# kleinzcy/speech_signal_processing

Measured on AMD Instinct MI355X. Metric: MFCC frames/s (one fused pass: framing .. DCT + delta + delta-delta, 39-d), higher is better.
Workload: dtype f32; 1 GPU; configs[1]: 100000 x 3 s synthetic 16 kHz utterances per GPU, 39-d MFCC (+delta+delta-delta), 400/160/512, 24 mel; utterances_per_gpu=100000, frames_per_gpu=29800000, d_out=39, parallelism=utterance-sharded x1, world_size_observed=1

## Files before the change

### speech_signal_processing_amd/csrc/mfcc.hpp

```cpp
#pragma once
#include "common.hpp"

namespace ssp {

struct MfccChunk {
    int32_t utt;
    int32_t t0;
    int32_t n;
    int32_t pad;
};

struct MfccArgs {
    const float* samples;
    const int64_t* sample_off;
    const int64_t* frame_off;
    float* out;
    float* lm_out;
    const MfccChunk* chunks;
    float* utt_max;
    const float* window;
    const float2* twiddle;
    const int32_t* filt_lo4;
    const float* filt_wT;
    const int32_t* filt_grp;
    int32_t filt_w4_total;
    int32_t dct_identity;
    int32_t dct_ncp;
    const float* dct;
    const float* dctT;
    int32_t win_len, hop, n_fft, n_filt, n_ceps, d_out;
    int32_t frame_mode, preemph_mode, spec_power, log_mode, floor_mode, delta_order, delta_N, cmvn;
    float preemph, spec_scale, eps, top_db, delta_inv_denom;
    int32_t lds_logmel_off, lds_ceps_off, lds_dlt_off, lds_ddl_off, lds_lmrows_off, lds_stats_off, lds_tw_off;
    int32_t lds_dct_off;
    int32_t lds_wt_off;
    int32_t lm_stride;
    int32_t n_chunks;
    int32_t prefetch;
};

constexpr int MFCC_FAST_MAX_PASS = 4;

struct FastArgs {
    const float2* tw16;
    const float2* wpost;
    const float* melw;
    const int32_t* mel_lo;
    const int32_t* mel_id;
    const float* dctT;
    int32_t mel_steps[MFCC_FAST_MAX_PASS];
    int32_t mel_blocks[MFCC_FAST_MAX_PASS];
    int32_t lm_pad;
    int32_t n_pass, q_pass, total_steps, n_filt4;
    float ddw[17];
    int32_t slen;
    int32_t stage_floats;
    int32_t ceps_rows;
    int32_t off_win, off_tw16, off_wpost, off_melw, off_mello, off_melid, off_dct, off_ceps, off_stats, off_wave, wave_bytes;
    float pscale;
    float one_minus_a;
    const float* pc_w;
    const int32_t* pc_ofs;
    const float* pc_mask;
    const int32_t* pc_fid;
    int32_t melv;
    int32_t mel_ns;
    float log_add, log_max, log_k;
    float* ceps_scratch;
    int32_t* work_counter;
    int32_t* redo_flags;
    int32_t ceps_stride;
    int32_t n_chunks;
};

struct StreamArgs {
    const float* dctA;
    int32_t* work_counter;
    int32_t* redo_flags;
    int32_t n_chunks;
    int32_t wave_bytes;
    int32_t stage_bytes;
    int32_t table_bytes;
    int32_t tstep;
    const float* dense_w;
};

int launch_mfcc_generic(const MfccArgs& args, int n_chunks, size_t lds_bytes, int n_waves, int num_cu, hipStream_t stream);
int launch_cmvn(const float* in, float* out, const int64_t* frame_off_dev, int64_t n_utt, int dim, int64_t max_T, hipStream_t stream);
int launch_topdb_dct(const float* logmel, const int64_t* frame_off_dev, int64_t n_utt, const MfccChunk* chunks, int n_chunks,
                     const float* utt_max, int n_filt, int n_ceps, const float* dct, float top_db, float* out, hipStream_t stream);
    

}

struct ssp_mfcc_plan {
    ssp_ctx* ctx = nullptr;
    ssp_mfcc_cfg cfg{};
    int32_t d_out = 0;
    bool reproducible = false;
    ssp::DevBuf window, twiddle, filt_lo4, filt_grp, filt_wT, dct, dctT, fbank_dense;
    int32_t max_filt_len = 0;
    uint64_t checked_sseg = 0, checked_fseg = 0;
    uint64_t cache_sseg = 0;
    uint64_t cache_fseg = 0;
    int cache_variant = -1;
    int cache_request = -1;
    bool cache_split_cmvn = false;
    bool cache_split_topdb = false;
    ssp::DevBuf lm_scratch, umax_scratch;
    int cache_chunk_frames = 0;
    size_t cache_lds = 0;
    int cache_waves = 4;
    int32_t cache_n_chunks = 0;
    std::vector<int32_t> cache_chunk_first;
    ssp::DevBuf chunks;
    ssp::MfccArgs args{};
    bool fast_ready = false;
    int64_t fast_max_samples = 0;
    ssp::FastArgs fast{};
    ssp::DevBuf f_tw16, f_wpost, f_melw, f_mello, f_melid, f_dct, f_pcw, f_pcofs, f_pcmask, f_pcfid, f_scratch, f_counter;
    bool stream_ready = false;
    ssp::DevBuf s_dctA, s_dense;
    bool cache_s2k_fused = false;
    bool s2k_ready = false;
    int32_t s2k_steps = 0, s2k_steps1 = 0;
    ssp::DevBuf s2k_twA, s2k_twB, s2k_twS, s2k_mel, s2k_minfo;
};

namespace ssp {
bool mfcc_fast_supported(const ssp_mfcc_cfg& cfg);
int build_fast_tables(ssp_mfcc_plan* plan);
size_t mfcc_fast_lds(const ssp_mfcc_cfg& cfg, FastArgs& f, int chunk_frames);
int mfcc_fast_max_chunk(const ssp_mfcc_cfg& cfg, const FastArgs& f);
int launch_mfcc_fast(const MfccArgs& args, ssp_mfcc_plan* plan, int n_chunks, int chunk_frames, hipStream_t stream);
bool mfcc_stream_supported(const ssp_mfcc_plan* plan);
bool mfcc_s2k_supported(const ssp_mfcc_plan* plan);
int build_s2k_tables(ssp_mfcc_plan* plan);
bool mfcc_s2k_fuses(const ssp_mfcc_plan* plan, int64_t max_T, int chunk_frames);
int launch_mfcc_s2k(const MfccArgs& args, ssp_mfcc_plan* plan, int n_chunks, hipStream_t stream);
bool mfcc_stream_dense(const ssp_mfcc_plan* plan);
bool mfcc_stream_fuses_cmvn(const ssp_mfcc_plan* plan);
int build_stream_tables(ssp_mfcc_plan* plan);
int launch_mfcc_stream(const MfccArgs& args, ssp_mfcc_plan* plan, int n_chunks, hipStream_t stream, bool dry_run = false);
}
```

### speech_signal_processing_amd/csrc/mfcc_plan.hip

```cpp
#include <chrono>
#include <cmath>
#include <cstdlib>

#include "mfcc.hpp"

namespace ssp {

static int validate_cfg(const ssp_mfcc_cfg* c) {
    if (!c) SSP_FAIL(SSP_ERR_INVALID, "mfcc: null cfg");
    if (c->n_fft < 64 || c->n_fft > 2048 || (c->n_fft & (c->n_fft - 1)))
        SSP_FAIL(SSP_ERR_UNSUPPORTED, "mfcc: n_fft=%d must be a power of two in [64, 2048]", c->n_fft);
    if (c->win_len < 1 || c->win_len > c->n_fft) SSP_FAIL(SSP_ERR_INVALID, "mfcc: win_len=%d not in [1, n_fft]", c->win_len);
    if (c->hop < 1) SSP_FAIL(SSP_ERR_INVALID, "mfcc: hop < 1");
    if (c->n_filt < 1 || c->n_filt > 512) SSP_FAIL(SSP_ERR_INVALID, "mfcc: n_filt=%d not in [1,512]", c->n_filt);
    if (c->n_ceps < 1 || c->n_ceps > 128) SSP_FAIL(SSP_ERR_INVALID, "mfcc: n_ceps=%d not in [1,128]", c->n_ceps);
    if (c->frame_mode < 0 || c->frame_mode > 2) SSP_FAIL(SSP_ERR_INVALID, "mfcc: frame_mode");
    if (c->frame_mode == 2 && c->win_len != c->n_fft)
        SSP_FAIL(SSP_ERR_UNSUPPORTED, "mfcc: centred framing needs win_len == n_fft");
    if (c->preemph_mode < 0 || c->preemph_mode > 1) SSP_FAIL(SSP_ERR_INVALID, "mfcc: preemph_mode");
    if (c->spec_power != 1 && c->spec_power != 2) SSP_FAIL(SSP_ERR_INVALID, "mfcc: spec_power must be 1 or 2");
    if (c->log_mode < 0 || c->log_mode > 2) SSP_FAIL(SSP_ERR_INVALID, "mfcc: log_mode");
    if (c->floor_mode < 0 || c->floor_mode > 2) SSP_FAIL(SSP_ERR_INVALID, "mfcc: floor_mode");
    if (c->delta_order < 0 || c->delta_order > 2) SSP_FAIL(SSP_ERR_INVALID, "mfcc: delta_order must be 0, 1 or 2");
    if (c->delta_order > 0 && (c->delta_N < 1 || c->delta_N > 8))
// ... 124 lines not shown
        if (whole) {
            ch = (int)std::max<int64_t>(max_T, 1);
            if (generic_lds_layout(c, ch, 8, &tmp) <= lds_cap) {
                nw = 8;
            } else if (generic_lds_layout(c, ch, 4, &tmp) > lds_cap) {
                if (c.top_db >= 0.f) {
                    if (c.delta_order != 0 || c.cmvn)
                        SSP_FAIL(SSP_ERR_UNSUPPORTED,
                                 "mfcc: top_db with deltas / cmvn needs a whole utterance per workgroup; %lld frames exceed the 160 KiB LDS",
                                 (long long)max_T);
                    split_topdb = true;
                } else {
                    split_cmvn = true;
                }
                whole = false;
                ch = chunk_for(c);
                if (split_topdb) {
                    ssp_mfcc_cfg c2 = c;
                    c2.top_db = -1.f;
                    ch = chunk_for(c2);
                }
            }
        }
        {
            ssp_mfcc_cfg c2 = c;
            if (split_topdb) c2.top_db = -1.f;
            lds = generic_lds_layout(c2, ch, nw, &p->args);
        }
        if (lds > lds_cap) SSP_FAIL(SSP_ERR_UNSUPPORTED, "mfcc: LDS footprint %zu B exceeds 160 KiB", lds);
    }
    std::vector<MfccChunk> chunks;
    chunks.reserve((size_t)fseg->n);
    int64_t tail_from = fseg->n;
#ifndef SSP_NO_TAIL_SPLIT
    if (variant == 3 && !(c.cmvn != 0 && !split_cmvn) && !getenv("SSP_MFCC_NO_TAIL_SPLIT")) {
        const int64_t waves = (int64_t)p->ctx->num_cu * 12;
        if (fseg->n >= 4 * waves) tail_from = fseg->n - waves;
    }
#endif
    p->cache_chunk_first.assign((size_t)fseg->n + 1, 0);
    for (int64_t u = 0; u < fseg->n; ++u) {
        const int64_t T = fseg->host[u + 1] - fseg->host[u];
        if (T > INT32_MAX) SSP_FAIL(SSP_ERR_UNSUPPORTED, "mfcc: utterance %lld has too many frames", (long long)u);
        p->cache_chunk_first[(size_t)u] = (int32_t)std::min<size_t>(chunks.size(), (size_t)INT32_MAX);
        int64_t chu = ch;
        if (u >= tail_from && T >= 64) chu = std::min<int64_t>(ch, ((T + 1) / 2 + 15) / 16 * 16);
        const int pad = (variant == 3 && (!small_batch || repro)) ? 12 : 0;
        for (int64_t t0 = 0; t0 < T; t0 += chu)
            chunks.push_back(MfccChunk{(int32_t)u, (int32_t)t0, (int32_t)std::min<int64_t>(chu, T - t0), t0 > 0 ? pad : 0});
    }
    if (chunks.size() > (size_t)INT32_MAX) SSP_FAIL(SSP_ERR_UNSUPPORTED, "mfcc: too many chunks");
    p->cache_chunk_first[(size_t)fseg->n] = (int32_t)chunks.size();
    SSP_TRY(upload(p->chunks, chunks, p->ctx->stream));
    SSP_HIP(hipStreamSynchronize(p->ctx->stream));
    p->fast_max_samples = sseg->max_len();
    p->cache_n_chunks = (int32_t)chunks.size();
    p->cache_chunk_frames = ch;
    p->cache_lds = lds;
    p->cache_waves = nw;
    p->cache_sseg = sseg->serial;
    p->cache_fseg = fseg->serial;
    p->cache_variant = variant;
    p->cache_split_cmvn = split_cmvn;
    p->cache_split_topdb = split_topdb;
    return SSP_OK;
}

}

using namespace ssp;

extern "C" {

int ssp_mfcc_num_frames(const ssp_mfcc_cfg* cfg, int64_t n_samples, int64_t* n_frames) {
    if (!cfg || !n_frames || n_samples < 0) SSP_FAIL(SSP_ERR_INVALID, "ssp_mfcc_num_frames: bad argument");
    if (cfg->hop < 1 || cfg->frame_mode < 0 || cfg->frame_mode > 2) SSP_FAIL(SSP_ERR_INVALID, "ssp_mfcc_num_frames: bad cfg");
    *n_frames = frames_for(*cfg, n_samples);
    return SSP_OK;
}

int ssp_mfcc_out_dim(const ssp_mfcc_cfg* cfg, int32_t* d_out) {
    if (!cfg || !d_out) SSP_FAIL(SSP_ERR_INVALID, "ssp_mfcc_out_dim: null");
    *d_out = cfg->n_ceps * (1 + cfg->delta_order);
    return SSP_OK;
}

int ssp_mfcc_plan_create(ssp_ctx* ctx, const ssp_mfcc_cfg* cfg, const float* window, const float* fbank,
                         const float* dct, ssp_mfcc_plan** out) {
    ssp::TraceRange trace_("ssp_mfcc_plan_create");
    if (!out) SSP_FAIL(SSP_ERR_INVALID, "ssp_mfcc_plan_create: null out");
    *out = nullptr;
    SSP_TRY(use_ctx(ctx));
    SSP_TRY(validate_cfg(cfg));
    if (!window || !fbank || !dct) SSP_FAIL(SSP_ERR_INVALID, "ssp_mfcc_plan_create: null table");
    ssp_mfcc_plan* p = new (std::nothrow) ssp_mfcc_plan;
    if (!p) SSP_FAIL(SSP_ERR_NOMEM, "mfcc plan: host alloc");
    p->ctx = ctx;
    p->cfg = *cfg;
    p->d_out = cfg->n_ceps * (1 + cfg->delta_order);
    const int n_fft = cfg->n_fft, nb = n_fft / 2 + 1;

    std::vector<float> win(n_fft, 0.f);
    for (int i = 0; i < cfg->win_len; ++i) win[i] = window[i];
    std::vector<float2> tw(n_fft);
    for (int k = 0; k < n_fft; ++k) {
        const double ang = -2.0 * M_PI * (double)k / (double)n_fft;
// ... 523 lines not shown
```

### speech_signal_processing_amd/csrc/mfcc_stream_kernel.hpp

```cpp
#pragma once
#include <algorithm>
#include <cmath>
#include <cstdlib>
#include <type_traits>

#include "mfcc.hpp"
#include "cplx.hpp"

namespace ssp {

namespace {
typedef unsigned v2u __attribute__((ext_vector_type(2)));
typedef __attribute__((address_space(3))) const volatile v2f* lds_cv2f_t;
typedef __attribute__((address_space(3))) const volatile float* lds_cvf_t;
constexpr int ZROW = 128;
constexpr int ZFRAME = 16 * ZROW;
constexpr int LM_OFF = 1792;
constexpr int RING_FRAMES = 24;
constexpr int RING_ROW = 64;
constexpr int STREAM_WAVES = 4;
#ifndef SSP_S_PSHIFT
#define SSP_S_PSHIFT 64
#endif
constexpr int PSH = SSP_S_PSHIFT;
static_assert(4 * (256 + 24) + PSH <= LM_OFF - 192, "shifted P row: piece reads must stay below the log-mel rows");
#define SSP_STR_(x) #x
#define SSP_STR(x) SSP_STR_(x)

__device__ __forceinline__ float stream_log(const FastArgs& f, float v) {
    return __builtin_amdgcn_logf(fmaxf(v + f.log_add, f.log_max)) * f.log_k;
}

__device__ __forceinline__ float delta_weight(float t, float tp, float Tm1, float half_inv) {
    const float lo = tp <= 0.f ? -1.0e6f : tp;
    const float hi = tp >= Tm1 ? 1.0e6f : tp;
    const float a = fmaxf(lo, t - 2.f), b = fminf(hi, t + 2.f);
    const float cnt = fmaxf(b - a + 1.f, 0.f);
    const float w = cnt * (a + b - 2.f * t) * half_inv;
    return (tp < 0.f || tp > Tm1) ? 0.f : w;
}
}

template <int NZ, int POWER, int PRE, int MELV, int KS, int NS, int OCC, int CM, int WALK, int GEO>
__device__ __forceinline__ void mfcc_stream512_body(const MfccArgs& a, const FastArgs& f, const StreamArgs& sa) {
    static_assert(GEO >= 0 && GEO <= 3 && (GEO == 0 || (NZ == 13 && KS == 6 && MELV != 0)), "fixed geometry: the 400 / 160 / 24-filter family only");
    constexpr bool FIXG = GEO != 0;
    extern __shared__ __attribute__((aligned(16))) char smem[];
    if (WALK && sa.work_counter[1] == 0) return;
    const int tid = threadIdx.x, lane = tid & 63;
    const int wave = __builtin_amdgcn_readfirstlane(tid >> 6);
    const int g = lane >> 4, j = lane & 15;
    constexpr int nc = 13;
    constexpr int mel_ns = NS;

    char* zbuf = smem + wave * sa.wave_bytes;
    float* stage = reinterpret_cast<float*>(zbuf + 4 * ZFRAME);
    char* ring = zbuf + 4 * ZFRAME + sa.stage_bytes;

    v2f wreg[NZ];
#pragma unroll
    for (int n1 = 0; n1 < NZ; ++n1) wreg[n1] = *reinterpret_cast<const v2f*>(a.window + 32 * n1 + 2 * j);
#pragma unroll
    for (int n1 = 0; n1 < NZ; ++n1) wreg[n1] = edge_row_taps(wreg[n1], 32 * n1 + 2 * j, a.win_len);
#ifndef SSP_STREAM_NTW
#define SSP_STREAM_NTW 15
#endif
#ifndef SSP_STREAM_NTW_CM
#define SSP_STREAM_NTW_CM 12
#endif
#ifndef SSP_STREAM_NWP
#define SSP_STREAM_NWP 8
#endif
    constexpr int NTW = OCC >= 3 ? (CM ? SSP_STREAM_NTW_CM : ((MELV <= 3 && NS <= 2) ? SSP_STREAM_NTW : ((MELV >= 4 && NS >= 4) ? 8 : 9))) : 15, NWP = OCC >= 3 ? SSP_STREAM_NWP : 8;
    static_assert(NTW >= 8, "rows above NTW take W^((k1 - 8) j) W^(8 j): W^(8 j) = twr[7] must be resident");
    v2f twr[NTW], wpr[NWP];
#pragma unroll
    for (int k1 = 1; k1 <= NTW; ++k1) twr[k1 - 1] = *reinterpret_cast<const v2f*>(&f.tw16[k1 * 16 + j]);
    float dA[KS];
#pragma unroll
    for (int s = 0; s < KS; ++s) dA[s] = sa.dctA[s * 64 + lane];
#pragma unroll
    for (int i = 0; i < NWP; ++i) wpr[i] = *reinterpret_cast<const v2f*>(&f.wpost[i * 16 + j]);
    constexpr bool DENSE = MELV == 0;
    constexpr int MV = DENSE ? 1 : MELV;
    v4f mw[MV];
    int mofs[MV];
    v2f mk01 = v2f{0.f, 0.f}, mk23 = v2f{0.f, 0.f};
    int mfid = -1;
    v4f dw[DENSE ? 6 : 1][4];
    float dw256[DENSE ? 6 : 1];
    if (DENSE) {
#pragma unroll
        for (int k = 0; k < 6; ++k) {
#pragma unroll
            for (int i = 0; i < 4; ++i) dw[DENSE ? k : 0][i] = *reinterpret_cast<const v4f*>(sa.dense_w + ((size_t)lane * 6 + k) * 20 + 4 * i);
            dw256[DENSE ? k : 0] = sa.dense_w[((size_t)lane * 6 + k) * 20 + 16];
        }
    } else {
#pragma unroll
        for (int i = 0; i < MV; ++i) {
            mw[i] = *reinterpret_cast<const v4f*>(f.pc_w + ((size_t)lane * MV + i) * 4);
            mofs[i] = f.pc_ofs[lane * MV + i];
        }
        mk01 = *reinterpret_cast<const v2f*>(f.pc_mask + lane * 4);
        mk23 = NS > 2 ? *reinterpret_cast<const v2f*>(f.pc_mask + lane * 4 + 2) : v2f{0.f, 0.f};
        mfid = f.pc_fid[lane];
    }

    const int hop = FIXG ? 160 : a.hop;
    const float pre = PRE ? a.preemph : 0.f;
    const float npre = -pre;
    const int slen = FIXG ? 3 * 160 + 32 * 13 : f.slen;
    const int n_piece = (slen + 255) >> 8;
    const bool has_half = (slen & 255) != 0 && (slen & 255) <= 128;
    const int n_full = has_half ? n_piece - 1 : n_piece;
    const int dord = FIXG ? GEO - 1 : a.delta_order;
    const int Dd = FIXG ? nc * GEO : a.d_out;
    const int n_filt = FIXG ? 24 : a.n_filt;
    const int lm_pad = FIXG ? 0 : f.lm_pad;
    const float half_inv = 0.5f * a.delta_inv_denom;
    const uint32_t stage_lds = __builtin_amdgcn_readfirstlane((uint32_t)(uintptr_t)(lds_ptr_t)stage);

#ifdef SSP_S_CLOCK
    const unsigned long long ck0 = __builtin_amdgcn_s_memtime(), rt0 = __builtin_amdgcn_s_memrealtime();
#endif
    uint64_t wm = 0;
    int wblk = blockIdx.x * STREAM_WAVES + wave, wbase = 0;
    for (;;) {
        int cidx = 0;
        if constexpr (WALK) {
            bool done = false;
            while (wm == 0) {
                if ((int64_t)wblk * 64 >= sa.n_chunks) {
                    done = true;
                    break;
                }
                const int idx = wblk * 64 + lane;
                const int fl = idx < sa.n_chunks ? sa.redo_flags[idx] : 0;
                wm = __builtin_amdgcn_ballot_w64(fl != 0);
                wbase = wblk * 64;
                wblk += gridDim.x * STREAM_WAVES;
            }
            if (done) break;
            cidx = __builtin_amdgcn_readfirstlane(wbase + __builtin_ctzll(wm));
            wm &= wm - 1;
        } else {
            if (lane == 0) cidx = atomicAdd(sa.work_counter, 1);
            cidx = __builtin_amdgcn_readfirstlane(cidx);
            if (cidx >= sa.n_chunks) break;
        }
        const MfccChunk ch = a.chunks[cidx];
        const int64_t s0 = a.sample_off[ch.utt];
        const int64_t N = a.sample_off[ch.utt + 1] - s0;
        const int64_t f0 = a.frame_off[ch.utt];
        const int T = __builtin_amdgcn_readfirstlane((int)(a.frame_off[ch.utt + 1] - f0));
        const int t0 = __builtin_amdgcn_readfirstlane(ch.t0), n = __builtin_amdgcn_readfirstlane(ch.n);
        const int H = dord > 0 ? 4 : 0;
        const int Hlo = dord > 0 ? H + __builtin_amdgcn_readfirstlane(ch.pad) : 0;
        const int ta = max(t0 - Hlo, 0), tb = min(t0 + n + H, T);
        const int R = tb - ta;
        const int nquads = (R + 3) >> 2;
        const int E = t0 + n - ta;
        const int n_steps = (E + 4 + 15) >> 4;
        const int Q = DENSE ? nquads : 4 * n_steps;
        const float Tm1 = (float)(T - 1);

        const uint64_t xaddr = reinterpret_cast<uint64_t>(a.samples + s0);
        const uint32_t xlo = __builtin_amdgcn_readfirstlane((uint32_t)xaddr), xhi = __builtin_amdgcn_readfirstlane((uint32_t)(xaddr >> 32));
        const int xbytes = __builtin_amdgcn_readfirstlane((int)(N * 4));
        const __amdgpu_buffer_rsrc_t rs = __builtin_amdgcn_make_buffer_rsrc(
            reinterpret_cast<float*>(((uint64_t)xhi << 32) | xlo), 0, xbytes, 0x00020000);
        const uint64_t oaddr = reinterpret_cast<uint64_t>(a.out + (size_t)f0 * Dd);
        const uint32_t olo = __builtin_amdgcn_readfirstlane((uint32_t)oaddr), ohi = __builtin_amdgcn_readfirstlane((uint32_t)(oaddr >> 32));
        const __amdgpu_buffer_rsrc_t ro = __builtin_amdgcn_make_buffer_rsrc(
            reinterpret_cast<float*>(((uint64_t)ohi << 32) | olo), 0, __builtin_amdgcn_readfirstlane(T * Dd * 4), 0x00020000);

        auto prefetch = [&](int q) {
            int ol = lane;
            if (FIXG) asm volatile("" : "+v"(ol));
            const int vo = (ta + 4 * q) * hop * 4 + ol * 16;
            const lds_ptr_t lp = (lds_ptr_t)(uintptr_t)stage_lds;
            if (FIXG) {
                __builtin_amdgcn_raw_ptr_buffer_load_lds(rs, lp, 16, vo, 0, 0, 0);
                __builtin_amdgcn_raw_ptr_buffer_load_lds(rs, lp, 16, vo, 0, 1024, 0);
                __builtin_amdgcn_raw_ptr_buffer_load_lds(rs, lp, 16, vo, 0, 2048, 0);
                if (lane < 32) __builtin_amdgcn_raw_ptr_buffer_load_lds(rs, lp, 16, vo, 0, 3072, 0);
                return;
            }
            if (n_full > 0) __builtin_amdgcn_raw_ptr_buffer_load_lds(rs, lp, 16, vo, 0, 0, 0);
            if (n_full > 1) __builtin_amdgcn_raw_ptr_buffer_load_lds(rs, lp, 16, vo, 0, 1024, 0);
            if (n_full > 2) __builtin_amdgcn_raw_ptr_buffer_load_lds(rs, lp, 16, vo, 0, 2048, 0);
            if (n_full > 3) __builtin_amdgcn_raw_ptr_buffer_load_lds(rs, lp, 16, vo, 0, 3072, 0);
            if (n_full > 4) __builtin_amdgcn_raw_ptr_buffer_load_lds(rs, (lds_ptr_t)(uintptr_t)(stage_lds + 4096), 16, vo + 4096, 0, 0, 0);
            if (has_half && lane < 32)
                __builtin_amdgcn_raw_ptr_buffer_load_lds(rs, (lds_ptr_t)(uintptr_t)(stage_lds + n_full * 1024), 16, vo + n_full * 1024, 0, 0, 0);
        };

        {
            float zz = 0.f;
            asm volatile("" : "+v"(zz));
            v4f z4 = v4f{zz, zz, zz, zz};
            *reinterpret_cast<v4f*>(ring + lane * 16) = z4;
            if (lane < (RING_FRAMES * RING_ROW - 1024) / 16) *reinterpret_cast<v4f*>(ring + 1024 + lane * 16) = z4;
        }
        prefetch(0);
        int stores_pending = 0;
        int cm_nf = WALK;
        float cs1[CM ? 3 : 1] = {}, cs2[CM ? 3 : 1] = {};
        float piv = 0.f;

        typedef v2f zarr_t[16];
        typedef v2f pfarr_t[NZ];
        typedef float pmarr_t[PRE ? NZ : 1];
        constexpr int NH = (NZ + 1) / 2;
        auto wait_dma = [&]() {
#ifndef SSP_S_NOWAIT
            if constexpr (FIXG) {
                if (__builtin_expect(stores_pending == 0, 1)) {
                    asm volatile("s_waitcnt vmcnt(0)" ::: "memory");
                } else {
                    int np = stores_pending;
                    asm volatile("" : "+s"(np));
// ... 126 lines not shown
                        if (POWER == 1) {
                            pa[u] = __builtin_amdgcn_sqrtf(pa[u]);
                            pb[u] = __builtin_amdgcn_sqrtf(pb[u]);
                        }
                    }
                    const int k2 = 2 * kp;
                    P[j + 16 * k2] = pa[0];
                    P[j + 16 * (k2 + 1)] = pa[1];
                    Pm[16 * (6 - k2)] = pb[1];
                    Pm[16 * (7 - k2)] = pb[0];
                }
                const v2f s8 = z[8] * z[8];
                float p128 = 4.f * (s8.x + s8.y);
                if (POWER == 1) p128 = __builtin_amdgcn_sqrtf(p128);
                if (j == 0) P[128] = p128;
            }
        };
        auto mel = [&]() {
#ifndef SSP_S_NOMEL
            if (!CM) {
                float* lm = reinterpret_cast<float*>(zbuf + g * ZFRAME + LM_OFF - 64 * g);
                if (j < lm_pad) lm[n_filt + j] = 0.f;
            } else if (j < lm_pad) {
                int ol = lane;
                asm volatile("" : "+v"(ol));
                reinterpret_cast<float*>(zbuf + (ol >> 4) * (ZFRAME - 64) + LM_OFF)[n_filt + (ol & 15)] = 0.f;
            }
            float sfr[4];
#pragma unroll
            for (int fr = 0; fr < 4; ++fr) {
                const char* pr = zbuf + fr * ZFRAME + (fr & 1) * PSH;
                v4f acc = *reinterpret_cast<const v4f*>(pr + mofs[0]) * mw[0];
#pragma unroll
                for (int i = 1; i < MV; ++i) acc = __builtin_elementwise_fma(*reinterpret_cast<const v4f*>(pr + mofs[i]), mw[i], acc);
                const v2f h = v2f{acc.x, acc.y} + v2f{acc.z, acc.w};
                sfr[fr] = h.x + h.y;
            }
            v2f s01 = v2f{sfr[0], sfr[1]}, s23 = v2f{sfr[2], sfr[3]};
#define SSP_SCAN_STEP(CTRL, MK)                                                                     \
            {                                                                                           \
                const float a0 = s01.x, a1 = s01.y, a2 = s23.x, a3 = s23.y;                             \
                const float b0 = __builtin_amdgcn_update_dpp(a0, a0, CTRL, 0xF, 0xF, true);           \
                const float b1 = __builtin_amdgcn_update_dpp(a1, a1, CTRL, 0xF, 0xF, true);           \
                const float b2 = __builtin_amdgcn_update_dpp(a2, a2, CTRL, 0xF, 0xF, true);           \
                const float b3 = __builtin_amdgcn_update_dpp(a3, a3, CTRL, 0xF, 0xF, true);           \
                s01 = __builtin_elementwise_fma(v2f{b0, b1}, MK, s01);                                  \
                s23 = __builtin_elementwise_fma(v2f{b2, b3}, MK, s23);                                  \
            }
            if (mel_ns > 0) SSP_SCAN_STEP(0x101 , xx(mk01))
            if (mel_ns > 1) SSP_SCAN_STEP(0x102 , yy(mk01))
            if (mel_ns > 2) SSP_SCAN_STEP(0x104 , xx(mk23))
            if (mel_ns > 3) SSP_SCAN_STEP(0x108 , yy(mk23))
#undef SSP_SCAN_STEP
            if (mfid >= 0) {
                float* lmf = reinterpret_cast<float*>(zbuf + LM_OFF) + mfid;
                lmf[0 * (ZFRAME - 64) / 4] = stream_log(f, s01.x);
                lmf[1 * (ZFRAME - 64) / 4] = stream_log(f, s01.y);
                lmf[2 * (ZFRAME - 64) / 4] = stream_log(f, s23.x);
                lmf[3 * (ZFRAME - 64) / 4] = stream_log(f, s23.y);
            }
#endif
        };
        auto dct_mfma = [&]() -> v4f {
            v4f cq = v4f{0.f, 0.f, 0.f, 0.f};
#ifndef SSP_S_NODCT
            int ol = lane;
            asm volatile("" : "+v"(ol));
            const int g = ol >> 4, j = ol & 15;
            const char* lmrow = zbuf + (j & 3) * (ZFRAME - 64) + LM_OFF + g * (KS * 4);
            float lb[KS];
#pragma unroll
            for (int s = 0; s < KS; s += 2) {
                const v2f v = *reinterpret_cast<const v2f*>(lmrow + 4 * s);
                lb[s] = v.x;
                lb[s + 1] = v.y;
            }
#pragma unroll
            for (int s = 0; s < KS; ++s) cq = __builtin_amdgcn_mfma_f32_16x16x4f32(dA[s], lb[s], cq, 0, 0, 0);
#endif
            return cq;
        };
        constexpr int RING_BYTES = RING_FRAMES * RING_ROW, QROW = 4 * RING_ROW;
        auto ring_wrap = [](int o) { return o >= RING_BYTES ? o - RING_BYTES : o; };
        int qrow = 0, srow = 0;
        auto ring_put = [&](int qq, v4f cq, bool real) {
            int ol = lane;
            asm volatile("" : "+v"(ol));
            const int g = ol >> 4, j = ol & 15;
            if (j < 4) {
                const bool ok = real && ta + 4 * qq + j < tb;
                const v4f cv = ok ? cq : v4f{0.f, 0.f, 0.f, 0.f};
                if constexpr (FIXG) *reinterpret_cast<v4f*>(ring + qrow + j * RING_ROW + g * 16) = cv;
                else *reinterpret_cast<v4f*>(ring + ((((qq + 6) % 6) * 4 + j) * RING_ROW) + g * 16) = cv;
            }
            if (FIXG) qrow = ring_wrap(qrow + QROW);
        };
        typedef float cbarr_t[6];
        auto ring_window = [&](int b, cbarr_t& cb) {
            const int rb = 16 * b;
            int ol = lane;
            asm volatile("" : "+v"(ol));
            const int g = ol >> 4, j = ol & 15;
            int mb = ring_wrap(srow + 16 * RING_ROW);
#pragma unroll
            for (int s = 0; s < 6; ++s) {
                if constexpr (FIXG) {
                    cb[s] = *reinterpret_cast<const float*>(ring + mb + g * RING_ROW + j * 4);
                    mb = ring_wrap(mb + QROW);
                } else {
                    const int m = (rb + 16 + 4 * s) % RING_FRAMES;
                    cb[s] = *reinterpret_cast<const float*>(ring + (m + g) * RING_ROW + j * 4);
                }
            }
        };
        auto time_step = [&](int b, const cbarr_t& cb) {
            const int rb = 16 * b;
            int ol = lane;
            asm volatile("" : "+v"(ol));
            const int g = ol >> 4, j = ol & 15;
            const float tg = (float)(ta + rb);
            const bool interior = ta + rb - 8 >= 1 && ta + rb + 16 <= T - 2;
            const float inv = 2.f * half_inv;
            auto W = [&](float tr, float tpr) -> float {
                if (interior) {
                    const float d = tpr - tr;
                    return __builtin_fabsf(d) <= 2.f ? d * inv : 0.f;
                }
                return delta_weight(tg + tr, tg + tpr, Tm1, half_inv);
            };
            const float fj = (float)j, fg = (float)g;
            const int Fo = ta + rb - 4 + 4 * g;
            const bool full = ta + rb - 4 >= t0 && ta + rb + 12 <= t0 + n;
            const int lane_off = j < nc ? (Fo * Dd + j) * 4 : 0x7ffffff0;
            auto put = [&](int rrel, int blk, float v, bool lane_on) {
                int off;
                if (full) {
                    off = lane_on ? lane_off + (rrel * Dd + blk * nc) * 4 : 0x7ffffff0;
                } else {
                    const int F = Fo + rrel;
                    off = (lane_on && F >= t0 && F < t0 + n) ? lane_off + (rrel * Dd + blk * nc) * 4 : 0x7ffffff0;
                }
#ifdef SSP_S_NOSTORE
                asm volatile("" ::"v"(v), "v"(off));
#else
                __builtin_amdgcn_raw_buffer_store_b32(__builtin_bit_cast(unsigned, v), ro, off, 0, 0);
#endif
                if (CM) {
                    const float dv = off != 0x7ffffff0 ? (blk == 0 ? v - piv : v) : 0.f;
// ... 220 lines not shown
                    window_b(z, pf, pm, std::integral_constant<int, 1>{});
                    fft_front(z);
                    mel();
                    const v4f cq = dct_mfma();
                    ring_put(q, cq, true);
                } else {
                    ring_put(q, v4f{0.f, 0.f, 0.f, 0.f}, false);
                }
                if ((q & 3) == 3) time_step_nf(q >> 2);
            }
        } else {
#ifdef SSP_S_SEQ
            for (int q = 0; q < Q; ++q) {
                zarr_t z;
                pfarr_t pf;
                pmarr_t pm;
                if (q < nquads) {
                    wait_dma();
                    stage_read_a(pf, pm);
                    asm volatile("s_waitcnt lgkmcnt(0)" ::: "memory");
                    window_a(z, pf, pm, std::integral_constant<int, DENSE ? 2 : 0>{});
                    stage_read_b(pf, pm);
                    asm volatile("s_waitcnt lgkmcnt(0)" ::: "memory");
#ifndef SSP_S_NODMA
                    prefetch(q + 1);
#endif
                    window_b(z, pf, pm, std::integral_constant<int, DENSE ? 2 : 0>{});
                    fft_front(z);
                    mel();
                    const v4f cq = dct_mfma();
                    ring_put(q, cq, true);
                } else {
                    ring_put(q, v4f{0.f, 0.f, 0.f, 0.f}, false);
                }
#ifndef SSP_S_NOSTEP
                if ((q & 3) == 3) emit_step(q >> 2);
#endif
            }
#else
#ifdef SSP_S_PAD
            asm volatile(".rept " SSP_STR(SSP_S_PAD) "\n s_nop 0\n .endr");
#endif
            if (FIXG) qrow = 5 * QROW;
            for (int q = 0; q < nquads; ++q) {
                zarr_t z;
                pfarr_t pf;
                pmarr_t pm;
                wait_dma();
                stage_read_a(pf, pm);
                const v4f cq = dct_mfma();
                asm volatile("s_waitcnt lgkmcnt(0)" ::: "memory");
                window_a(z, pf, pm, std::integral_constant<int, DENSE ? 2 : 0>{});
                stage_read_b(pf, pm);
                ring_put(q - 1, cq, q > 0);
                asm volatile("s_waitcnt lgkmcnt(0)" ::: "memory");
#ifndef SSP_S_NODMA
                prefetch(q + 1);
#endif
                window_b(z, pf, pm, std::integral_constant<int, DENSE ? 2 : 0>{});
                fft_front(z);
                mel();
#ifndef SSP_S_NOSTEP
                if ((q & 3) == 0 && q > 0) emit_step((q - 1) >> 2);
#endif
            }
            for (int qb = nquads - 1; qb < Q; ++qb) {
                v4f cq = v4f{0.f, 0.f, 0.f, 0.f};
                if (qb < nquads) cq = dct_mfma();
                ring_put(qb, cq, qb < nquads);
#ifndef SSP_S_NOSTEP
                if ((qb & 3) == 3) emit_step(qb >> 2);
#endif
            }
#endif
        }
        asm volatile("s_waitcnt vmcnt(0)" ::: "memory");
        if (CM) {
            int ol = lane;
            asm volatile("" : "+v"(ol));
            const int g = ol >> 4, j = ol & 15;
            float* ct = reinterpret_cast<float*>(ring);
            if (cm_nf) {
                double n1 = 0.0, a1 = 0.0, a2 = 0.0;
                const int col = ol < Dd ? ol : 0;
                for (int F0 = 0; F0 < T; F0 += 8) {
                    float v[8];
#pragma unroll
                    for (int k = 0; k < 8; ++k)
                        v[k] = __builtin_bit_cast(float, __builtin_amdgcn_raw_buffer_load_b32(ro, F0 + k < T ? ((F0 + k) * Dd + col) * 4 : 0x7ffffff0, 0, 1));
#pragma unroll
                    for (int k = 0; k < 8; ++k) {
                        const bool ok = F0 + k < T && v[k] == v[k];
                        const double d = ok ? (double)v[k] : 0.0;
                        n1 += ok ? 1.0 : 0.0;
                        a1 += d;
                        a2 += d * d;
                    }
                }
                const double mean = a1 / n1;
                const double var = a2 / n1 - mean * mean;
                double sd = __builtin_sqrt(var > 0.0 ? var : (var == var ? 0.0 : var));
                if (sd < 10.0 * 1.1920929e-07) sd = 1.0;
                if (ol < Dd) {
                    ct[ol] = (float)mean;
                    ct[48 + ol] = (float)(1.0 / sd);
                }
            } else
#pragma unroll
            for (int blk = 0; blk < 3; ++blk) {
                if (blk > dord) break;
                double a1 = (double)cs1[CM ? blk : 0], a2 = (double)cs2[CM ? blk : 0];
                auto xor_add = [&](double v, int m) -> double {
                    const v2u b = __builtin_bit_cast(v2u, v);
                    const int addr = (ol ^ m) << 2;
                    const v2u o = v2u{(unsigned)__builtin_amdgcn_ds_bpermute(addr, (int)b.x), (unsigned)__builtin_amdgcn_ds_bpermute(addr, (int)b.y)};
                    return v + __builtin_bit_cast(double, o);
                };
                a1 = xor_add(a1, 16);
                a2 = xor_add(a2, 16);
                a1 = xor_add(a1, 32);
                a2 = xor_add(a2, 32);
                const double m0 = a1 / (double)T;
                const double mean = m0 + (blk == 0 ? (double)piv : 0.0);
                const double var = a2 / (double)T - m0 * m0;
                double sd = __builtin_sqrt(var > 0.0 ? var : (var == var ? 0.0 : var));
                if (sd < 10.0 * 1.1920929e-07) sd = 1.0;
                if (g == 0 && j < nc) {
                    ct[blk * nc + j] = (float)mean;
// ... 22 lines not shown
                        const int off = idx < n_el ? idx * (4 * W) : 0x7ffffff0;
                        const int c1 = c + 1 == Dd ? 0 : c + 1;
                        const float m0 = ct[c], is0 = ct[48 + c];
                        if (W == 2) {
                            const float m1 = ct[c1], is1 = ct[48 + c1];
                            const v2f o = v2f{(v[k].x - m0) * is0, (v[k].y - m1) * is1};
                            __builtin_amdgcn_raw_buffer_store_b64(__builtin_bit_cast(v2u, o), ro, off, 0, 0);
                        } else {
                            __builtin_amdgcn_raw_buffer_store_b32(__builtin_bit_cast(unsigned, (v[k].x - m0) * is0), ro, off, 0, 0);
                        }
                        c += step;
                        c = c >= Dd ? c - Dd : c;
                    }
                }
            };
            if ((Dd & 1) == 0) rewrite(std::integral_constant<int, 2>{});
            else rewrite(std::integral_constant<int, 1>{});
            asm volatile("s_waitcnt vmcnt(0) lgkmcnt(0)" ::: "memory");
        }
    }
#ifdef SSP_S_CLOCK
    if (tid == 0) {
        const unsigned long long ck1 = __builtin_amdgcn_s_memtime(), rt1 = __builtin_amdgcn_s_memrealtime();
        atomicAdd(reinterpret_cast<unsigned long long*>(sa.work_counter + 8), ck1 - ck0);
        atomicAdd(reinterpret_cast<unsigned long long*>(sa.work_counter + 10), rt1 - rt0);
    }
#endif
}

template <int NZ, int POWER, int PRE, int MELV, int KS, int NS, int OCC, int CM, int WALK>
__global__ __launch_bounds__(64 * STREAM_WAVES, OCC) void mfcc_stream512_kernel(MfccArgs a, FastArgs f, StreamArgs sa) {
    mfcc_stream512_body<NZ, POWER, PRE, MELV, KS, NS, OCC, CM, WALK, 0>(a, f, sa);
}
template <int NZ, int POWER, int PRE, int MELV, int KS, int NS, int OCC, int CM, int WALK, int GEO>
__global__ __launch_bounds__(64 * STREAM_WAVES, OCC) void mfcc_stream512_geo_kernel(MfccArgs a, FastArgs f, StreamArgs sa) {
    static_assert(GEO >= 1, "GEO = 0 is mfcc_stream512_kernel");
    mfcc_stream512_body<NZ, POWER, PRE, MELV, KS, NS, OCC, CM, WALK, GEO>(a, f, sa);
}
constexpr bool stream_geo_excluded(int melv, int ns, int cm, int geo) { return geo == 2 && cm == 0 && melv == 3 && ns <= 2; }
typedef void (*stream_kernel_t)(MfccArgs, FastArgs, StreamArgs);
template <int NZ, int POWER, int PRE, int MELV, int KS, int NS, int OCC, int CM, int WALK, int GEO>
static inline stream_kernel_t stream_kernel() {
    if constexpr (GEO == 0) return mfcc_stream512_kernel<NZ, POWER, PRE, MELV, KS, NS, OCC, CM, WALK>;
    else if constexpr (stream_geo_excluded(MELV, NS, CM, GEO)) return nullptr;
    else return mfcc_stream512_geo_kernel<NZ, POWER, PRE, MELV, KS, NS, OCC, CM, WALK, GEO>;
}

static inline int stream_ks(const ssp_mfcc_cfg& c) { return (c.n_filt + 3) / 4 <= 6 ? 6 : 10; }

static inline bool stream_fixed_geo(const ssp_mfcc_cfg& c, const FastArgs& f, const MfccArgs& a) {
    if (getenv("SSP_MFCC_STREAM_RUNTIME_GEO")) return false;
    return c.win_len == 400 && c.hop == 160 && a.hop == 160 && c.n_filt == 24 && a.n_filt == 24 && c.n_ceps == 13 && c.spec_power == 2 &&
           c.preemph_mode != 0 && f.slen == 3 * 160 + 32 * 13 && f.melv >= 2 && f.melv <= 4 && a.delta_order >= 0 && a.delta_order <= 2 &&
           a.d_out == 13 * (1 + a.delta_order);
}

template <int WALK>
int launch_mfcc_stream_impl(const MfccArgs& args, ssp_mfcc_plan* p, int n_chunks, hipStream_t stream, bool dry_run) {
    if (n_chunks <= 0 && !dry_run) return SSP_OK;
    FastArgs f = p->fast;
    const ssp_mfcc_cfg& c = p->cfg;
    StreamArgs sa{};
    const int KS = stream_ks(c);
    f.lm_pad = 4 * KS - c.n_filt;
    if (f.lm_pad > 16 && f.melv != 0) SSP_FAIL(SSP_ERR_UNSUPPORTED, "mfcc(stream): %d filters leave more than 16 padded slots", c.n_filt);
    sa.dctA = p->s_dctA.as<float>();
    sa.dense_w = p->s_dense.as<float>();
    const int n_piece = (f.slen + 255) >> 8;
    const bool has_half = (f.slen & 255) != 0 && (f.slen & 255) <= 128;
    sa.stage_bytes = has_half ? (n_piece - 1) * 1024 + 512 : n_piece * 1024;
    sa.wave_bytes = 4 * ZFRAME + sa.stage_bytes + RING_FRAMES * RING_ROW;
    sa.table_bytes = 0;
    sa.n_chunks = n_chunks;
    if (!dry_run) {
        SSP_TRY(p->f_counter.reserve(64 + (size_t)std::max(n_chunks, 1) * sizeof(int32_t)));
        sa.work_counter = p->f_counter.as<int32_t>();
        sa.redo_flags = sa.work_counter + 16;
    }
    size_t lds = (size_t)sa.table_bytes + (size_t)STREAM_WAVES * sa.wave_bytes;
    if (const char* e = getenv("SSP_MFCC_LDS_PAD")) lds = std::min<size_t>(160 * 1024, lds + (size_t)atoi(e));
    if (lds > 160 * 1024) SSP_FAIL(SSP_ERR_UNSUPPORTED, "mfcc(stream): LDS footprint %zu B exceeds 160 KiB", lds);
    if ((int64_t)p->fast_max_samples * 4 > INT32_MAX) SSP_FAIL(SSP_ERR_UNSUPPORTED, "mfcc(stream): utterance too long for 32-bit offsets");
    const int nz = c.win_len <= 416 ? 13 : 16, pw = c.spec_power, pr = c.preemph_mode ? 1 : 0;
    const int cm = args.cmvn != 0 ? 1 : 0;
    const int occ = (nz == 13 && KS == 6 && lds <= 53248 && f.melv != 0 && (!cm || (f.melv <= 3 && f.mel_ns <= 2))) ? 3 : 2;
    const int wg_waves = STREAM_WAVES;
#ifdef SSP_FAST_MINIMAL
    const bool geo_inst = f.melv == 3 && f.mel_ns <= 2 && !cm && occ == 3;
#else
    const bool geo_inst = cm || occ == 3;
#endif
    const int geo = (stream_fixed_geo(c, f, args) && KS == 6 && nz == 13 && sa.stage_bytes == 3 * 1024 + 512 && geo_inst &&
                     !stream_geo_excluded(f.melv, f.mel_ns <= 2 ? 2 : 4, cm, 1 + args.delta_order)) ? 1 + args.delta_order : 0;
    bool launched = false;
#define SSP_STREAM_CASE(NZ_, PW_, PR_, MV_, KS_, OCC_) SSP_STREAM_CASE_CM(NZ_, PW_, PR_, MV_, KS_, OCC_, 0)
#define SSP_STREAM_CASE_CM(NZ_, PW_, PR_, MV_, KS_, OCC_, CM_) SSP_STREAM_CASE_G(NZ_, PW_, PR_, MV_, KS_, OCC_, CM_, 0)
#define SSP_STREAM_CASE_G(NZ_, PW_, PR_, MV_, KS_, OCC_, CM_, GEO_)                                                   \
    if (!launched && dry_run && nz == NZ_ && pw == PW_ && pr == PR_ && f.melv == MV_ && KS == KS_ && occ == OCC_ && cm == CM_ && geo == GEO_) \
        launched = true;                                                                                                \
    if (!launched && nz == NZ_ && pw == PW_ && pr == PR_ && f.melv == MV_ && KS == KS_ && occ == OCC_ && cm == CM_ && geo == GEO_) { \
        const stream_kernel_t kfn = f.mel_ns <= 2 ? stream_kernel<NZ_, PW_, PR_, MV_, KS_, 2, OCC_, CM_, WALK, GEO_>()    \
                                                  : stream_kernel<NZ_, PW_, PR_, MV_, KS_, 4, OCC_, CM_, WALK, GEO_>();   \
        if (lds > 64 * 1024)                                                                                            \
            SSP_HIP(hipFuncSetAttribute(reinterpret_cast<const void*>(kfn), hipFuncAttributeMaxDynamicSharedMemorySize, (int)lds)); \
        int per_cu = 0;                                                                                                 \
        SSP_HIP(hipOccupancyMaxActiveBlocksPerMultiprocessor(&per_cu, kfn, 64 * wg_waves, lds));                        \
        const int grid = std::min((n_chunks + wg_waves - 1) / wg_waves, std::max(1, per_cu) * p->ctx->num_cu);          \
        if (!WALK) SSP_HIP(hipMemsetAsync(sa.work_counter, 0, 64 + (size_t)n_chunks * 4, stream));     \
        if (getenv("SSP_DEBUG")) fprintf(stderr, "[ssp] mfcc stream%s: grid %d (%d per CU), lds %zu, geo %d cm %d\n", WALK ? " (second kernel)" : "", grid, per_cu, lds, GEO_, CM_); \
        hipLaunchKernelGGL(kfn, dim3(grid), dim3(64 * wg_waves), lds, stream, args, f, sa);                             \
        launched = true;                                                                                                \
    }
#define SSP_STREAM_CASE_CM3(MV_, GEO_)                                                                                    \
    if (!launched && dry_run && nz == 13 && pw == 2 && pr == 1 && f.melv == MV_ && KS == 6 && occ == 3 && cm == 1 && geo == GEO_) launched = true; \
    if (!launched && nz == 13 && pw == 2 && pr == 1 && f.melv == MV_ && KS == 6 && occ == 3 && cm == 1 && geo == GEO_) {    \
        const stream_kernel_t kfn = stream_kernel<13, 2, 1, MV_, 6, 2, 3, 1, WALK, GEO_>();                               \
        int per_cu = 0;                                                                                                   \
        SSP_HIP(hipOccupancyMaxActiveBlocksPerMultiprocessor(&per_cu, kfn, 64 * wg_waves, lds));                          \
        const int grid = std::min((n_chunks + wg_waves - 1) / wg_waves, std::max(1, per_cu) * p->ctx->num_cu);            \
        if (!WALK) SSP_HIP(hipMemsetAsync(sa.work_counter, 0, 64 + (size_t)n_chunks * 4, stream));                            \
        if (getenv("SSP_DEBUG")) fprintf(stderr, "[ssp] mfcc stream%s: grid %d (%d per CU), lds %zu, geo %d cm 1\n", WALK ? " (second kernel)" : "", grid, per_cu, lds, GEO_); \
        hipLaunchKernelGGL(kfn, dim3(grid), dim3(64 * wg_waves), lds, stream, args, f, sa);                               \
        launched = true;                                                                                                  \
    }
    SSP_STREAM_CASE_CM3(2, 0) SSP_STREAM_CASE_CM3(3, 0)
    SSP_STREAM_CASE_CM(13, 2, 1, 2, 6, 2, 1) SSP_STREAM_CASE_CM(13, 2, 1, 3, 6, 2, 1) SSP_STREAM_CASE_CM(13, 2, 1, 4, 6, 2, 1)
#ifdef SSP_FAST_MINIMAL
    SSP_STREAM_CASE_G(13, 2, 1, 3, 6, 3, 0, 1) SSP_STREAM_CASE_G(13, 2, 1, 3, 6, 3, 0, 3)
#else
#define SSP_STREAM_FIXED(GEO_)                                                                                            \
    SSP_STREAM_CASE_CM3(2, GEO_) SSP_STREAM_CASE_CM3(3, GEO_)                                                             \
    SSP_STREAM_CASE_G(13, 2, 1, 2, 6, 2, 1, GEO_) SSP_STREAM_CASE_G(13, 2, 1, 3, 6, 2, 1, GEO_) SSP_STREAM_CASE_G(13, 2, 1, 4, 6, 2, 1, GEO_) \
    SSP_STREAM_CASE_G(13, 2, 1, 2, 6, 3, 0, GEO_) SSP_STREAM_CASE_G(13, 2, 1, 3, 6, 3, 0, GEO_) SSP_STREAM_CASE_G(13, 2, 1, 4, 6, 3, 0, GEO_)
    SSP_STREAM_FIXED(1) SSP_STREAM_FIXED(2) SSP_STREAM_FIXED(3)
#undef SSP_STREAM_FIXED
#endif
#undef SSP_STREAM_CASE_CM3
    if constexpr (!WALK) {
        SSP_STREAM_CASE(13, 2, 1, 0, 6, 2)
    }
#ifdef SSP_FAST_MINIMAL
    SSP_STREAM_CASE(13, 2, 1, 3, 6, 3)
    SSP_STREAM_CASE(16, 1, 0, 3, 10, 2)
    SSP_STREAM_CASE(16, 1, 0, 5, 10, 2)
#else
#define SSP_STREAM_MV(NZ_, PW_, PR_, KS_, OCC_)                                                                         \
// ... 26 lines not shown
```

Measured before the change: 3.151 billion frames/s.

## Claim next stream chunk ahead with packed scalar records; drop log floor and ring index math

Adds a packed 32-byte per-chunk record table built on the host, so each wave fetches its chunk metadata with a single scalar load. The atomic work claim and record fetch for the next chunk are issued at the end of the current chunk, hiding their latency behind the output drain. It also drops the log floor/clamp when the config has no floor, and replaces the modulo-based ring row index with an incremental pointer. This costs an extra table upload and makes the fixed-geometry path depend on the records being present.

```diff
diff --git a/speech_signal_processing_amd/csrc/mfcc.hpp b/speech_signal_processing_amd/csrc/mfcc.hpp
--- a/speech_signal_processing_amd/csrc/mfcc.hpp
+++ b/speech_signal_processing_amd/csrc/mfcc.hpp
@@ -9,6 +9,16 @@
     int32_t n;
     int32_t pad;
 };
+
+struct StreamChunkRec {
+    int64_t s0;
+    int64_t f0;
+    int32_t xbytes;
+    int32_t T;
+    int32_t t0;
+    int32_t n_pad;
+};
+static_assert(sizeof(StreamChunkRec) == 32, "one s_load_dwordx8 per chunk");
 
 struct MfccArgs {
     const float* samples;
@@ -83,6 +93,7 @@
     int32_t table_bytes;
     int32_t tstep;
     const float* dense_w;
+    const StreamChunkRec* chunk_rec;
 };
 
 int launch_mfcc_generic(const MfccArgs& args, int n_chunks, size_t lds_bytes, int n_waves, int num_cu, hipStream_t stream);
@@ -114,6 +125,7 @@
     int32_t cache_n_chunks = 0;
     std::vector<int32_t> cache_chunk_first;
     ssp::DevBuf chunks;
+    ssp::DevBuf chunk_rec;
     ssp::MfccArgs args{};
     bool fast_ready = false;
     int64_t fast_max_samples = 0;
diff --git a/speech_signal_processing_amd/csrc/mfcc_plan.hip b/speech_signal_processing_amd/csrc/mfcc_plan.hip
--- a/speech_signal_processing_amd/csrc/mfcc_plan.hip
+++ b/speech_signal_processing_amd/csrc/mfcc_plan.hip
@@ -200,6 +200,16 @@
     if (chunks.size() > (size_t)INT32_MAX) SSP_FAIL(SSP_ERR_UNSUPPORTED, "mfcc: too many chunks");
     p->cache_chunk_first[(size_t)fseg->n] = (int32_t)chunks.size();
     SSP_TRY(upload(p->chunks, chunks, p->ctx->stream));
+    std::vector<StreamChunkRec> recs;
+    if (variant == 3) {
+        recs.reserve(chunks.size());
+        for (const MfccChunk& k : chunks) {
+            const int64_t s0 = sseg->host[(size_t)k.utt], N = sseg->host[(size_t)k.utt + 1] - s0;
+            const int64_t f0 = fseg->host[(size_t)k.utt], T = fseg->host[(size_t)k.utt + 1] - f0;
+            recs.push_back(StreamChunkRec{s0, f0, (int32_t)std::min<int64_t>(N * 4, INT32_MAX), (int32_t)T, k.t0, k.n | (k.pad << 16)});
+        }
+        SSP_TRY(upload(p->chunk_rec, recs, p->ctx->stream));
+    }
     SSP_HIP(hipStreamSynchronize(p->ctx->stream));
     p->fast_max_samples = sseg->max_len();
     p->cache_n_chunks = (int32_t)chunks.size();
diff --git a/speech_signal_processing_amd/csrc/mfcc_stream_kernel.hpp b/speech_signal_processing_amd/csrc/mfcc_stream_kernel.hpp
--- a/speech_signal_processing_amd/csrc/mfcc_stream_kernel.hpp
+++ b/speech_signal_processing_amd/csrc/mfcc_stream_kernel.hpp
@@ -24,6 +24,15 @@
 #endif
 constexpr int PSH = SSP_S_PSHIFT;
 static_assert(4 * (256 + 24) + PSH <= LM_OFF - 192, "shifted P row: piece reads must stay below the log-mel rows");
+#ifndef SSP_S_NOFLOOR
+#define SSP_S_NOFLOOR 1
+#endif
+#ifndef SSP_S_PUTSC
+#define SSP_S_PUTSC 1
+#endif
+#ifndef SSP_S_AHEAD
+#define SSP_S_AHEAD 1
+#endif
 #define SSP_STR_(x) #x
 #define SSP_STR(x) SSP_STR_(x)
 
@@ -126,6 +135,20 @@
 #endif
     uint64_t wm = 0;
     int wblk = blockIdx.x * STREAM_WAVES + wave, wbase = 0;
+    constexpr bool AHEAD = FIXG && !WALK && SSP_S_AHEAD;
+    typedef int rec_t __attribute__((ext_vector_type(8)));
+    int nx_cidx = 0;
+    rec_t nx_rec = rec_t{0, 0, 0, 0, 0, 0, 0, 0};
+    auto claim_ahead = [&]() {
+        const __amdgpu_buffer_rsrc_t rc = __builtin_amdgcn_make_buffer_rsrc(sa.work_counter, 0, 4, 0x00020000);
+        int ol = lane;
+        asm volatile("" : "+v"(ol));
+        const int got = __builtin_amdgcn_raw_ptr_buffer_atomic_add_i32(1, rc, ol == 0 ? 0 : 0x7ffffff0, 0, 0);
+        nx_cidx = __builtin_amdgcn_readfirstlane(got);
+        const StreamChunkRec* rp = sa.chunk_rec + min(nx_cidx, sa.n_chunks - 1);
+        asm volatile("s_load_dwordx8 %0, %1, 0x0\n\ts_waitcnt lgkmcnt(0)" : "=&s"(nx_rec) : "s"(rp) : "memory");
+    };
+    if constexpr (AHEAD) claim_ahead();
     for (;;) {
         int cidx = 0;
         if constexpr (WALK) {
@@ -144,17 +167,33 @@
             if (done) break;
             cidx = __builtin_amdgcn_readfirstlane(wbase + __builtin_ctzll(wm));
             wm &= wm - 1;
+        } else if constexpr (AHEAD) {
+            cidx = nx_cidx;
+            if (cidx >= sa.n_chunks) break;
         } else {
             if (lane == 0) cidx = atomicAdd(sa.work_counter, 1);
             cidx = __builtin_amdgcn_readfirstlane(cidx);
             if (cidx >= sa.n_chunks) break;
         }
-        const MfccChunk ch = a.chunks[cidx];
-        const int64_t s0 = a.sample_off[ch.utt];
-        const int64_t N = a.sample_off[ch.utt + 1] - s0;
-        const int64_t f0 = a.frame_off[ch.utt];
-        const int T = __builtin_amdgcn_readfirstlane((int)(a.frame_off[ch.utt + 1] - f0));
-        const int t0 = __builtin_amdgcn_readfirstlane(ch.t0), n = __builtin_amdgcn_readfirstlane(ch.n);
+        MfccChunk ch{};
+        int64_t s0, N = 0, f0;
+        int T, t0, n, rec_xbytes = 0;
+        if constexpr (AHEAD) {
+            s0 = (int64_t)(((uint64_t)(uint32_t)nx_rec[1] << 32) | (uint32_t)nx_rec[0]);
+            f0 = (int64_t)(((uint64_t)(uint32_t)nx_rec[3] << 32) | (uint32_t)nx_rec[2]);
+            rec_xbytes = nx_rec[4];
+            T = nx_rec[5];
+            t0 = nx_rec[6];
+            n = nx_rec[7] & 0xffff;
+            ch.pad = nx_rec[7] >> 16;
+        } else {
+            ch = a.chunks[cidx];
+            s0 = a.sample_off[ch.utt];
+            N = a.sample_off[ch.utt + 1] - s0;
+            f0 = a.frame_off[ch.utt];
+            T = __builtin_amdgcn_readfirstlane((int)(a.frame_off[ch.utt + 1] - f0));
+            t0 = __builtin_amdgcn_readfirstlane(ch.t0), n = __builtin_amdgcn_readfirstlane(ch.n);
+        }
         const int H = dord > 0 ? 4 : 0;
         const int Hlo = dord > 0 ? H + __builtin_amdgcn_readfirstlane(ch.pad) : 0;
         const int ta = max(t0 - Hlo, 0), tb = min(t0 + n + H, T);
@@ -167,7 +206,7 @@
 
         const uint64_t xaddr = reinterpret_cast<uint64_t>(a.samples + s0);
         const uint32_t xlo = __builtin_amdgcn_readfirstlane((uint32_t)xaddr), xhi = __builtin_amdgcn_readfirstlane((uint32_t)(xaddr >> 32));
-        const int xbytes = __builtin_amdgcn_readfirstlane((int)(N * 4));
+        const int xbytes = AHEAD ? rec_xbytes : __builtin_amdgcn_readfirstlane((int)(N * 4));
         const __amdgpu_buffer_rsrc_t rs = __builtin_amdgcn_make_buffer_rsrc(
             reinterpret_cast<float*>(((uint64_t)xhi << 32) | xlo), 0, xbytes, 0x00020000);
         const uint64_t oaddr = reinterpret_cast<uint64_t>(a.out + (size_t)f0 * Dd);
@@ -400,12 +439,16 @@
             if (mel_ns > 2) SSP_SCAN_STEP(0x104 , xx(mk23))
             if (mel_ns > 3) SSP_SCAN_STEP(0x108 , yy(mk23))
 #undef SSP_SCAN_STEP
+            auto slog = [&](float v) -> float {
+                if constexpr (FIXG && SSP_S_NOFLOOR) return __builtin_amdgcn_logf(v) * f.log_k;
+                else return stream_log(f, v);
+            };
             if (mfid >= 0) {
                 float* lmf = reinterpret_cast<float*>(zbuf + LM_OFF) + mfid;
-                lmf[0 * (ZFRAME - 64) / 4] = stream_log(f, s01.x);
-                lmf[1 * (ZFRAME - 64) / 4] = stream_log(f, s01.y);
-                lmf[2 * (ZFRAME - 64) / 4] = stream_log(f, s23.x);
-                lmf[3 * (ZFRAME - 64) / 4] = stream_log(f, s23.y);
+                lmf[0 * (ZFRAME - 64) / 4] = slog(s01.x);
+                lmf[1 * (ZFRAME - 64) / 4] = slog(s01.y);
+                lmf[2 * (ZFRAME - 64) / 4] = slog(s23.x);
+                lmf[3 * (ZFRAME - 64) / 4] = slog(s23.y);
             }
 #endif
         };
@@ -442,6 +485,13 @@
                 else *reinterpret_cast<v4f*>(ring + ((((qq + 6) % 6) * 4 + j) * RING_ROW) + g * 16) = cv;
             }
             if (FIXG) qrow = ring_wrap(qrow + QROW);
+        };
+        auto ring_put_inner = [&](v4f cq, bool on) {
+            int ol = lane;
+            asm volatile("" : "+v"(ol));
+            const int g = ol >> 4, j = ol & 15;
+            if (j < 4 && on) *reinterpret_cast<v4f*>(ring + qrow + j * RING_ROW + g * 16) = cq;
+            qrow = ring_wrap(qrow + QROW);
         };
         typedef float cbarr_t[6];
         auto ring_window = [&](int b, cbarr_t& cb) {
@@ -768,7 +818,8 @@
                 asm volatile("s_waitcnt lgkmcnt(0)" ::: "memory");
                 window_a(z, pf, pm, std::integral_constant<int, DENSE ? 2 : 0>{});
                 stage_read_b(pf, pm);
-                ring_put(q - 1, cq, q > 0);
+                if constexpr (FIXG && SSP_S_PUTSC) ring_put_inner(cq, q > 0);
+                else ring_put(q - 1, cq, q > 0);
                 asm volatile("s_waitcnt lgkmcnt(0)" ::: "memory");
 #ifndef SSP_S_NODMA
                 prefetch(q + 1);
@@ -790,6 +841,7 @@
             }
 #endif
         }
+        if constexpr (AHEAD) claim_ahead();
         asm volatile("s_waitcnt vmcnt(0)" ::: "memory");
         if (CM) {
             int ol = lane;
@@ -918,7 +970,8 @@
     if (getenv("SSP_MFCC_STREAM_RUNTIME_GEO")) return false;
     return c.win_len == 400 && c.hop == 160 && a.hop == 160 && c.n_filt == 24 && a.n_filt == 24 && c.n_ceps == 13 && c.spec_power == 2 &&
            c.preemph_mode != 0 && f.slen == 3 * 160 + 32 * 13 && f.melv >= 2 && f.melv <= 4 && a.delta_order >= 0 && a.delta_order <= 2 &&
-           a.d_out == 13 * (1 + a.delta_order);
+           a.d_out == 13 * (1 + a.delta_order) &&
+           (!SSP_S_NOFLOOR || (c.floor_mode == 0 && f.log_add == 0.f && f.log_max == -INFINITY));
 }
 
 template <int WALK>
@@ -932,6 +985,7 @@
     if (f.lm_pad > 16 && f.melv != 0) SSP_FAIL(SSP_ERR_UNSUPPORTED, "mfcc(stream): %d filters leave more than 16 padded slots", c.n_filt);
     sa.dctA = p->s_dctA.as<float>();
     sa.dense_w = p->s_dense.as<float>();
+    sa.chunk_rec = (p->chunk_rec.p && args.chunks) ? p->chunk_rec.as<StreamChunkRec>() + (args.chunks - p->chunks.as<MfccChunk>()) : nullptr;
     const int n_piece = (f.slen + 255) >> 8;
     const bool has_half = (f.slen & 255) != 0 && (f.slen & 255) <= 128;
     sa.stage_bytes = has_half ? (n_piece - 1) * 1024 + 512 : n_piece * 1024;
@@ -958,6 +1012,7 @@
 #endif
     const int geo = (stream_fixed_geo(c, f, args) && KS == 6 && nz == 13 && sa.stage_bytes == 3 * 1024 + 512 && geo_inst &&
                      !stream_geo_excluded(f.melv, f.mel_ns <= 2 ? 2 : 4, cm, 1 + args.delta_order)) ? 1 + args.delta_order : 0;
+    if (!dry_run && !WALK && geo != 0 && SSP_S_AHEAD && !sa.chunk_rec) SSP_FAIL(SSP_ERR_INVALID, "mfcc(stream): the work table has no chunk records");
     bool launched = false;
 #define SSP_STREAM_CASE(NZ_, PW_, PR_, MV_, KS_, OCC_) SSP_STREAM_CASE_CM(NZ_, PW_, PR_, MV_, KS_, OCC_, 0)
 #define SSP_STREAM_CASE_CM(NZ_, PW_, PR_, MV_, KS_, OCC_, CM_) SSP_STREAM_CASE_G(NZ_, PW_, PR_, MV_, KS_, OCC_, CM_, 0)
```

Result: faster. 3.193 billion frames/s (median of 6 runs) (+1.3%).
